# menmitsu/opticalFlowClustering

Measured on AMD Instinct MI355X. Metric: Mpixels/s dense flow+kmeans @1080p, higher is better.
Workload: dtype f32 storage, f64 accumulation; 1 GPU; BASELINE.json configs[2]: 300-frame 1080p synthetic clip, Farneback flow (0.5,3,15,3,5,1.2,0) + Lloyd k=5 over (u,v), frames sharded over 1 GPU(s); width=1920, height=1080, frames=300, pairs=299, k=5, lloyd_iters=11, flow_batch_pairs=64

## Files before the change

include/ofc.h:

```cpp
#ifndef OFC_H
#define OFC_H
#include <stddef.h>
#include <stdint.h>

#ifdef __cplusplus
extern "C" {
#endif

#define OFC_VERSION 100

enum {
    OFC_OK = 0,
    OFC_EINVAL = -1,
    OFC_ENODEV = -2,
    OFC_EHIP = -3,
    OFC_ENOMEM = -4,
    OFC_ENOTREADY = -5,
    OFC_EUNSUPPORTED = -6,
    OFC_ECOMM = -7
};

enum { OFC_U8 = 0, OFC_F32 = 1, OFC_F64 = 2 };

int ofc_version(void);
const char *ofc_last_error(void);
int ofc_device_count(int *n);

int ofc_malloc(int device, size_t bytes, void **dptr);
int ofc_free(int device, void *dptr);
int ofc_memcpy_h2d(int device, void *dst_dev, const void *src_host, size_t bytes);
int ofc_memcpy_d2h(int device, void *dst_host, const void *src_dev, size_t bytes);
int ofc_memset(int device, void *dst_dev, int value, size_t bytes);
int ofc_device_sync(int device);

typedef struct ofc_fb_params {
    double pyr_scale;
    int levels;
    int winsize;
    int iterations;
    int poly_n;
    double poly_sigma;
    int flags;
} ofc_fb_params;
#define OFC_WINSIZE_MAX 255

void ofc_fb_default_params(ofc_fb_params *p);

typedef struct ofc_flow ofc_flow_t;

int ofc_flow_create(int device, int W, int H, const ofc_fb_params *p, int max_batch,
                    ofc_flow_t **out);
void ofc_flow_destroy(ofc_flow_t *f);

int ofc_flow_calc(ofc_flow_t *f, const uint8_t *prev_gray, const uint8_t *next_gray,
                  float *flow_out);

int ofc_flow_calc_frames_dev(ofc_flow_t *f, const uint8_t *frames_dev, int n_frames,
                             float *flow_dev);
int ofc_flow_calc_frames_dev_stats(ofc_flow_t *f, const uint8_t *frames_dev, int n_frames,
                                   float *flow_dev, double *uv_sum_dev);
int ofc_flow_sync(ofc_flow_t *f);

int ofc_flow_push_gray(ofc_flow_t *f, const uint8_t *gray, float *flow_out);

int ofc_flow_push_bgr(ofc_flow_t *f, const uint8_t *bgr, uint8_t *vis_out, float *mean_mag,
                      float *flow_out);
int ofc_flow_last_vis_dev(ofc_flow_t *f, const uint8_t **vis_dev);

int ofc_level_image(int device, const uint8_t *gray, int W, int H, const ofc_fb_params *p, int k,
                    float *out, int *w_out, int *h_out);
int ofc_polyexp(int device, const float *img, int W, int H, int n, double sigma, float *R5);
int ofc_polyexp_u8(int device, const uint8_t *gray, int W, int H, int n, double sigma, float *R5);
int ofc_update_matrices(int device, const float *R0, const float *R1, const float *flow, int W,
                        int H, float *M);
int ofc_box_solve(int device, const float *M, int W, int H, int winsize, float *flow);
int ofc_flow_resize(int device, const float *flow, int sw, int sh, int dw, int dh, float mul,
                    float *out);

int ofc_flow_iterate(int device, const float *R0, const float *R1, const float *flow_in, int W, int H,
                     int winsize, int iters, int mode, int rows_per_block, float *flow_out);
int ofc_flow_launch_geometry(int W, int H, int n_pairs, int winsize, int out[3]);
int ofc_bench_flow_iters(int device, int W, int H, int n_pairs, int reps, int mode, float *ms);

int ofc_bench_polyexp(int device, int W, int H, int n_images, int iters, int rows_per_block,
                      float *ms_per_launch);

int ofc_bgr2gray(int device, const uint8_t *bgr, int W, int H, uint8_t *gray);
int ofc_flow_to_bgr(int device, const float *flow, int W, int H, uint8_t *bgr, float *mean_mag);
int ofc_flow_to_bgr_dev(int device, const float *flow_dev, int W, int H, int n_frames,
                        uint8_t *bgr_dev, float *mean_mag_dev);
int ofc_bgr2hsv(int device, const uint8_t *bgr, int64_t npix, uint8_t *hsv);
int ofc_preprocess_rgba(int device, const uint8_t *img3, int64_t npix, int thresh, uint8_t *rgba);
int ofc_grid_cell_means(int device, const uint8_t *bgr, int W, int H, int rows, int cols,
                        uint8_t *mean_bgr, uint8_t *hsv);

int ofc_kmeans_fit(int device, const void *X, int dtype, int64_t N, int d, int k,
                   const double *init, int max_iter, double tol_rel, double *centers,
                   int32_t *labels, double *inertia, int *n_iter);
int ofc_kmeans_predict(int device, const void *X, int dtype, int64_t N, int d, int k,
                       const double *centers, int32_t *labels);
int ofc_kmeans_fit_dev(int device, const void *X_dev, int dtype, int64_t N, int d, int k,
                       const double *init, int max_iter, double tol_rel, double *centers,
                       uint8_t *labels_dev, double *inertia, int *n_iter);
int ofc_kmeans_fit_dev_stats(int device, const void *X_dev, int dtype, int64_t N, int d, int k,
                             const double *init, int max_iter, double tol_rel, const double *colsum,
                             double *centers, uint8_t *labels_dev, double *inertia, int *n_iter);
int ofc_kmeans_fit_dev_field(int device, const void *X_dev, int dtype, int64_t N, int d, int k,
                             const double *init, int max_iter, double tol_rel, const double *colsum,
                             double *centers, uint8_t *labels_dev, double *inertia, int *n_iter,
                             int W, int H, int64_t n_fields);
int64_t ofc_lloyd_field_origin(int64_t tile, int quad, int W);
int ofc_lloyd_field_origins(int64_t tile0, int64_t n_tiles, int W, int64_t *out);
void ofc_lloyd_field_shape(int *tile_w, int *tile_h, int *group_w, int *group_h);
int ofc_lloyd_prune_stats(int device, double *out6);
int ofc_bench_lloyd_sweep(int device, const float *X_dev, int64_t N, int k, const double *centers, const double *mean,
                          int what, int iters, float *ms_per_launch);
int ofc_lloyd_colstats_dev(int device, const void *X_dev, int dtype, int64_t N, int d, const double *mean,
                           int pass, double *out);
int ofc_lloyd_step_dev(int device, const void *X_dev, int dtype, int64_t N, int d, int k, const double *mean,
                       const double *centers_c, uint8_t *labels_dev, int accumulate, double *record);
int ofc_lloyd_inertia_dev(int device, const void *X_dev, int dtype, int64_t N, int d, int k, const double *mean,
                          const double *centers_c, const uint8_t *labels_dev, double *inertia);
int ofc_lloyd_farthest_dev(int device, const void *X_dev, int dtype, int64_t N, int d, int k, const double *mean,
                           const double *centers_c, const uint8_t *labels_dev, const int64_t *excl, int n_excl,
                           double *dist2, int64_t *index, double *x_c, int *label);

int ofc_kmeans_fit_w(int device, const void *X, int dtype, const void *w, int w_dtype, int64_t N, int d, int k,
                     const double *init, int max_iter, double tol_rel, double *centers, int32_t *labels,
                     double *inertia, int *n_iter);
int ofc_kmeans_fit_dev_w(int device, const void *X_dev, int dtype, const void *w_dev, int w_dtype, int64_t N, int d,
                         int k, const double *init, int max_iter, double tol_rel, const double *colsum,
                         double *centers, uint8_t *labels_dev, double *inertia, int *n_iter);
int ofc_kmeans_score(int device, const void *X, int dtype, const void *w, int w_dtype, int64_t N, int d, int k,
                     const double *centers, double *inertia);
int ofc_lloyd_step_dev_w(int device, const void *X_dev, int dtype, const void *w_dev, int w_dtype, int64_t N, int d,
                         int k, const double *mean, const double *centers_c, uint8_t *labels_dev, double *record);
int ofc_lloyd_inertia_dev_w(int device, const void *X_dev, int dtype, const void *w_dev, int w_dtype, int64_t N, int d,
                            int k, const double *mean, const double *centers_c, const uint8_t *labels_dev,
                            double *inertia);
int ofc_lloyd_farthest_dev_w(int device, const void *X_dev, int dtype, const void *w_dev, int w_dtype, int64_t N, int d,
                             int k, const double *mean, const double *centers_c, const uint8_t *labels_dev,
                             const int64_t *excl, int n_excl, double *dist2, int64_t *index, double *x_c, int *label,
                             double *weight);
int ofc_flow_weights_dev(int device, const float *flow_dev, int64_t n, int kind, float thr, float *w_dev);
// ... 173 lines not shown
```

opticalflowclustering_amd/_lib.py:

```python
import ctypes as C
import os

import numpy as np

_HERE = os.path.dirname(os.path.abspath(__file__))
LIB_PATH = os.path.join(_HERE, "libofc.so")

OFC_OK, OFC_EINVAL, OFC_ENODEV, OFC_EHIP, OFC_ENOMEM, OFC_ENOTREADY, OFC_EUNSUPPORTED, OFC_ECOMM = \
    0, -1, -2, -3, -4, -5, -6, -7
U8, F32, F64 = 0, 1, 2
UNIQUE_ID_BYTES = 128
KPP_CHUNK = 1024
UV_HIST_SHARE = 2048
UV_HIST_MAX_GRID = 2048
BLOB_TILE_W, BLOB_TILE_H, BLOB_FIELDS = 64, 16, 12
BLOB_LINK_FIELDS, BLOB_NO_MOVE = 3, -0x7fff8000
CONSIST_OK, CONSIST_MISMATCH, CONSIST_LEAVES, CONSIST_INVALID, CONSIST_STATES = 0, 1, 2, 3, 4
CONSIST_SHARE, CONSIST_MAX_DIM = 2048, 16384
CONSIST_ALPHA_MAX, CONSIST_BETA_MAX = 65536, 1 << 62
PHOTO_SHARE, PHOTO_TAU_MAX, PHOTO_KAPPA_MAX, PHOTO_NSTAT = 2048, 65280, 1024, 5
REPAIR_ROUNDS_MAX, REPAIR_NCOUNT, REPAIR_UNFILLED = 254, 3, 255


class OfcError(RuntimeError):
    def __init__(self, code, msg):
        super().__init__(f"libofc error {code}: {msg}")
        self.code = code


class FbParams(C.Structure):
    _fields_ = [("pyr_scale", C.c_double), ("levels", C.c_int), ("winsize", C.c_int),
                ("iterations", C.c_int), ("poly_n", C.c_int), ("poly_sigma", C.c_double),
                ("flags", C.c_int)]

    def __init__(self, pyr_scale=0.5, levels=3, winsize=15, iterations=3, poly_n=5, poly_sigma=1.2,
                 flags=0):
        super().__init__(pyr_scale, levels, winsize, iterations, poly_n, poly_sigma, flags)


_lib = None

_vp, _i, _i64, _f, _d, _sz = C.c_void_p, C.c_int, C.c_int64, C.c_float, C.c_double, C.c_size_t
_ip = C.POINTER(C.c_int)
_PROTOS = {
    "ofc_version": ([], _i),
    "ofc_last_error": ([], C.c_char_p),
    "ofc_device_count": ([_ip], _i),
    "ofc_malloc": ([_i, _sz, C.POINTER(_vp)], _i),
    "ofc_free": ([_i, _vp], _i),
    "ofc_memcpy_h2d": ([_i, _vp, _vp, _sz], _i),
    "ofc_memcpy_d2h": ([_i, _vp, _vp, _sz], _i),
    "ofc_memset": ([_i, _vp, _i, _sz], _i),
    "ofc_device_sync": ([_i], _i),
    "ofc_fb_default_params": ([C.POINTER(FbParams)], None),
    "ofc_flow_create": ([_i, _i, _i, C.POINTER(FbParams), _i, C.POINTER(_vp)], _i),
    "ofc_flow_destroy": ([_vp], None),
    "ofc_flow_calc": ([_vp, _vp, _vp, _vp], _i),
    "ofc_flow_calc_frames_dev": ([_vp, _vp, _i, _vp], _i),
    "ofc_flow_calc_frames_dev_stats": ([_vp, _vp, _i, _vp, _vp], _i),
    "ofc_flow_sync": ([_vp], _i),
    "ofc_flow_push_gray": ([_vp, _vp, _vp], _i),
    "ofc_flow_push_bgr": ([_vp, _vp, _vp, C.POINTER(_f), _vp], _i),
    "ofc_flow_last_vis_dev": ([_vp, C.POINTER(_vp)], _i),
    "ofc_level_image": ([_i, _vp, _i, _i, C.POINTER(FbParams), _i, _vp, _ip, _ip], _i),
    "ofc_polyexp": ([_i, _vp, _i, _i, _i, _d, _vp], _i),
    "ofc_polyexp_u8": ([_i, _vp, _i, _i, _i, _d, _vp], _i),
    "ofc_update_matrices": ([_i, _vp, _vp, _vp, _i, _i, _vp], _i),
    "ofc_box_solve": ([_i, _vp, _i, _i, _i, _vp], _i),
    "ofc_flow_resize": ([_i, _vp, _i, _i, _i, _i, _f, _vp], _i),
    "ofc_flow_iterate": ([_i, _vp, _vp, _vp, _i, _i, _i, _i, _i, _i, _vp], _i),
    "ofc_flow_launch_geometry": ([_i, _i, _i, _i, _ip], _i),
    "ofc_bench_flow_iters": ([_i, _i, _i, _i, _i, _i, C.POINTER(_f)], _i),
    "ofc_bench_polyexp": ([_i, _i, _i, _i, _i, _i, C.POINTER(_f)], _i),
    "ofc_bgr2gray": ([_i, _vp, _i, _i, _vp], _i),
    "ofc_flow_to_bgr": ([_i, _vp, _i, _i, _vp, C.POINTER(_f)], _i),
    "ofc_flow_to_bgr_dev": ([_i, _vp, _i, _i, _i, _vp, _vp], _i),
    "ofc_bgr2hsv": ([_i, _vp, _i64, _vp], _i),
    "ofc_preprocess_rgba": ([_i, _vp, _i64, _i, _vp], _i),
    "ofc_grid_cell_means": ([_i, _vp, _i, _i, _i, _i, _vp, _vp], _i),
    "ofc_kmeans_fit": ([_i, _vp, _i, _i64, _i, _i, _vp, _i, _d, _vp, _vp, C.POINTER(_d), _ip], _i),
    "ofc_kmeans_predict": ([_i, _vp, _i, _i64, _i, _i, _vp, _vp], _i),
    "ofc_kmeans_fit_dev": ([_i, _vp, _i, _i64, _i, _i, _vp, _i, _d, _vp, _vp, C.POINTER(_d), _ip], _i),
    "ofc_kmeans_fit_dev_stats": ([_i, _vp, _i, _i64, _i, _i, _vp, _i, _d, _vp, _vp, _vp, C.POINTER(_d), _ip], _i),
    "ofc_kmeans_fit_dev_field": ([_i, _vp, _i, _i64, _i, _i, _vp, _i, _d, _vp, _vp, _vp, C.POINTER(_d), _ip, _i, _i, _i64], _i),
    "ofc_lloyd_field_origin": ([_i64, _i, _i], _i64),
    "ofc_lloyd_field_origins": ([_i64, _i64, _i, _vp], _i),
    "ofc_lloyd_field_shape": ([_ip, _ip, _ip, _ip], None),
    "ofc_lloyd_prune_stats": ([_i, _vp], _i),
    "ofc_bench_lloyd_sweep": ([_i, _vp, _i64, _i, _vp, _vp, _i, _i, C.POINTER(_f)], _i),
    "ofc_lloyd_colstats_dev": ([_i, _vp, _i, _i64, _i, _vp, _i, _vp], _i),
    "ofc_lloyd_step_dev": ([_i, _vp, _i, _i64, _i, _i, _vp, _vp, _vp, _i, _vp], _i),
    "ofc_lloyd_inertia_dev": ([_i, _vp, _i, _i64, _i, _i, _vp, _vp, _vp, C.POINTER(_d)], _i),
    "ofc_lloyd_farthest_dev": ([_i, _vp, _i, _i64, _i, _i, _vp, _vp, _vp, _vp, _i, C.POINTER(_d), C.POINTER(_i64), _vp, _ip], _i),
    "ofc_kmeans_fit_w": ([_i, _vp, _i, _vp, _i, _i64, _i, _i, _vp, _i, _d, _vp, _vp, C.POINTER(_d), _ip], _i),
    "ofc_kmeans_fit_dev_w": ([_i, _vp, _i, _vp, _i, _i64, _i, _i, _vp, _i, _d, _vp, _vp, _vp, C.POINTER(_d), _ip], _i),
    "ofc_kmeans_score": ([_i, _vp, _i, _vp, _i, _i64, _i, _i, _vp, C.POINTER(_d)], _i),
    "ofc_lloyd_step_dev_w": ([_i, _vp, _i, _vp, _i, _i64, _i, _i, _vp, _vp, _vp, _vp], _i),
    "ofc_lloyd_inertia_dev_w": ([_i, _vp, _i, _vp, _i, _i64, _i, _i, _vp, _vp, _vp, C.POINTER(_d)], _i),
    "ofc_lloyd_farthest_dev_w": ([_i, _vp, _i, _vp, _i, _i64, _i, _i, _vp, _vp, _vp, _vp, _i, C.POINTER(_d), C.POINTER(_i64), _vp, _ip,
                                  C.POINTER(_d)], _i),
    "ofc_flow_weights_dev": ([_i, _vp, _i64, _i, _f, _vp], _i),
    "ofc_bench_lloyd_sweep_w": ([_i, _vp, _vp, _i, _i64, _i, _vp, _vp, _i, C.POINTER(_f)], _i),
    "ofc_kpp_candidates": ([_i, _vp, _i, _i64, _i, _vp, _vp, _i, _vp, _vp, _vp], _i),
    "ofc_kpp_seed_dev": ([_i, _vp, _i, _i64, _i, _i, _vp, _i64, _vp, _i, _vp, _vp], _i),
    "ofc_kpp_sample_dev": ([_i, _vp, _i64, _vp, _i, _vp], _i),
    "ofc_kpp_seed_dev_w": ([_i, _vp, _i, _vp, _i, _i64, _i, _i, _vp, _d, _vp, _i, _vp, _vp], _i),
    "ofc_kpp_sample_dev_w": ([_i, _vp, _i, _vp, _i64, _vp, _i, _i, _vp, _vp], _i),
    "ofc_kmeans_fit_batched": ([_i, _vp, _vp, _i, _i, _i, _vp, _i, _d, _vp, _vp, _vp, _vp], _i),
    "ofc_grid_kmeans": ([_i, _vp, _i, _i, _i, _i, _i, _vp, _i, _d, _i, _vp, _vp], _i),
    "ofc_grid_kmeans_dev": ([_i, _vp, _i, _i, _i, _i, _i, _i, _vp, _i, _d, _i, _vp, _vp], _i),
    "ofc_dist_unique_id": ([_vp], _i),
    "ofc_dist_init": ([_i, _i, _i, _vp], _i),
    "ofc_dist_allreduce_f64": ([_i, _vp, _i], _i),
    "ofc_dist_init_host": ([_i, _i, _i, _vp, _vp], _i),
    "ofc_dist_loopback": ([_i], _i),
    "ofc_dist_finalize": ([], _i),
    "ofc_stream_create": ([_i, _i, _i, C.POINTER(FbParams), _i, _i, _i, C.POINTER(_vp)], _i),
    "ofc_stream_push_gray": ([_vp, _vp, _ip], _i),
    "ofc_stream_finish": ([_vp, _vp, _i, _ip], _i),
    "ofc_stream_set_model": ([_vp, _i, _vp, _vp, _i], _i),
    "ofc_stream_finish_clusters": ([_vp, _vp, _vp, _vp, _i, _ip], _i),
    "ofc_stream_set_histogram": ([_vp, _i, _f], _i),
    "ofc_stream_read_histogram": ([_vp, _vp, _i], _i),
    "ofc_stream_destroy": ([_vp], None),
    "ofc_grid_cell_mean_flow": ([_i, _vp, _i, _i, _i, _i, _vp], _i),
    "ofc_grid_label_counts_dev": ([_i, _vp, _vp, _i, _i, _i, _i, _i, _i, _vp, _vp], _i),
    "ofc_grid_assign_counts_dev": ([_i, _vp, _i, _i, _i, _i, _i, _i, _vp, _vp, _vp, _vp], _i),
    "ofc_uv_hist_accum_dev": ([_i, _vp, _i64, _i, _f, _vp], _i),
    "ofc_uv_hist": ([_i, _vp, _i64, _i, _f, _vp], _i),
    "ofc_bench_uv_hist": ([_i, _vp, _i64, _i, _f, _i, C.POINTER(_f)], _i),
    "ofc_motion_check": ([_i, _i, _i], _i),
    "ofc_motion_launch_geometry": ([_i, _i, _i, _ip], _i),
    "ofc_motion_solve": ([_vp, _i, _vp, _ip], _i),
    "ofc_motion_moments_dev": ([_i, _vp, _i, _i, _i, _vp, _vp, _vp], _i),
    "ofc_motion_fit_dev": ([_i, _vp, _i, _i, _i, _i, _vp, _i, _vp, _vp, _vp, _vp], _i),
    "ofc_motion_subtract_dev": ([_i, _vp, _i, _i, _i, _vp, _vp], _i),
    "ofc_motion_fit": ([_i, _vp, _i, _i, _i, _i, _vp, _i, _vp, _vp, _vp, _vp], _i),
    "ofc_motion_compensate": ([_i, _vp, _i, _i, _i, _i, _vp, _i, _vp, _vp, _vp, _vp, _vp], _i),
    "ofc_stream_set_camera": ([_vp, _i, _vp, _i], _i),
    "ofc_stream_read_camera": ([_vp, _vp, _vp, _i], _i),
    "ofc_bench_motion": ([_i, _vp, _i, _i, _i, _i, _i, C.POINTER(_f)], _i),
    "ofc_blob_check": ([_i, _i, _i, _i, _i, _i], _i),
    "ofc_blob_keys_dev": ([_i, _vp, _i, _i, _i, _i, _f, _i, _vp, _vp, C.c_uint32, _i, _vp], _i),
# ... 108 lines not shown
```

opticalflowclustering_amd/csrc/ofc_api.cpp:

```cpp
#include "color_common.h"
#include "lloyd_common.h"

#include <cfloat>
#include <algorithm>
#include <cmath>
#include <cstdlib>
#include <memory>

namespace ofc {

static thread_local std::string g_err;

void set_error(const char *fmt, ...)
{
    char buf[1024];
    va_list ap;
    va_start(ap, fmt);
    vsnprintf(buf, sizeof(buf), fmt, ap);
    va_end(ap);
    g_err = buf;
}

int ensure_device(int device)
{
// ... 109 lines not shown
        set_error("winsize %d unsupported (odd 5..%d)", p.winsize, OFC_WINSIZE_MAX);
        return OFC_EUNSUPPORTED;
    }
    return polyexp_n_check(p.poly_n);
}

}

using namespace ofc;

extern "C" {

int ofc_version(void) { return OFC_VERSION; }
const char *ofc_last_error(void) { return g_err.c_str(); }

int ofc_device_count(int *n)
{
    OFC_REQUIRE(n, "null pointer");
    int c = 0;
    hipError_t e = hipGetDeviceCount(&c);
    *n = (e == hipSuccess) ? c : 0;
    return OFC_OK;
}

int ofc_malloc(int device, size_t bytes, void **dptr)
{
    OFC_REQUIRE(dptr, "null pointer");
    OFC_TRY(ensure_device(device));
    OFC_HIP(hipMalloc(dptr, bytes));
    return OFC_OK;
}

int ofc_free(int device, void *dptr)
{
    OFC_TRY(ensure_device(device));
    OFC_HIP(hipFree(dptr));
    return OFC_OK;
}

int ofc_memcpy_h2d(int device, void *dst, const void *src, size_t bytes)
{
    OFC_TRY(ensure_device(device));
    OFC_HIP(hipMemcpy(dst, src, bytes, hipMemcpyHostToDevice));
    return OFC_OK;
}

int ofc_memcpy_d2h(int device, void *dst, const void *src, size_t bytes)
{
    OFC_TRY(ensure_device(device));
    OFC_HIP(hipMemcpy(dst, src, bytes, hipMemcpyDeviceToHost));
    return OFC_OK;
}

int ofc_memset(int device, void *dst, int value, size_t bytes)
{
    OFC_TRY(ensure_device(device));
    OFC_HIP(hipMemset(dst, value, bytes));
    return OFC_OK;
}

int ofc_device_sync(int device)
{
    OFC_TRY(ensure_device(device));
    OFC_HIP(hipDeviceSynchronize());
    return OFC_OK;
}

void ofc_fb_default_params(ofc_fb_params *p)
{
    if (!p) return;
    p->pyr_scale = 0.5; p->levels = 3; p->winsize = 15; p->iterations = 3;
    p->poly_n = 5; p->poly_sigma = 1.2; p->flags = 0;
}

}

struct ofc_flow {
    int device = 0, W = 0, H = 0, max_batch = 0, levels = 0;
    ofc_fb_params prm{};
    PolyConsts pc{};
    std::vector<LevelGeom> geom;
    hipStream_t stream = nullptr;
    DevBuf I, R, M, flowA, flowB, flowC;
    bool fused = true;
    bool fuse_level0 = true;
    bool fuse2 = false;
    int fuse2_min_w = 0;
    bool w3 = false;
    int w3_min_w = 0;
    DevBuf frames2, flow1;
    DevBuf prev_gray;
    bool have_prev = false;
    DevBuf bgr_in, vis, vis_partial, vis_stats, mean_mag;
    bool have_vis = false;
    DevBuf uv_scratch;
    struct Captured {
        const uint8_t *frames = nullptr;
        int n_frames = 0;
        float *flow = nullptr;
        double *uv_sum = nullptr;
        int hits = 0;
        hipGraph_t graph = nullptr;
        hipGraphExec_t exec = nullptr;
    };
    std::vector<Captured> graphs;
    bool use_graph = false;
};

namespace ofc {

static int flow_run(ofc_flow *f, const uint8_t *frames_dev, int n_frames, float *flow_dev, double *uv_sum_dev = nullptr)
{
    const int npair = n_frames - 1;
    const int W = f->W, H = f->H;
    hipStream_t s = f->stream;
    float *I = f->I.as<float>(), *R = f->R.as<float>();
    const int iters = f->prm.iterations;
    float *prevFlow = nullptr;
    int pw = 0, ph = 0;
    for (int k = f->levels; k >= 0; k--) {
        const LevelGeom &g = f->geom[k];
        const size_t P = (size_t)g.w * g.h;
        float *dst = (k == 0) ? flow_dev : (((f->levels - k) & 1) ? f->flowB.as<float>() : f->flowA.as<float>());
        float *tmp = f->flowC.as<float>();
        if (k == 0 && f->fuse_level0 && polyexp_u8_ok(W, H, g)) {
            OFC_TRY(launch_polyexp_u8(frames_dev, R, n_frames, W, H, f->pc, s));
        } else {
            OFC_TRY(launch_level_image(frames_dev, I, n_frames, W, H, g, s));
            OFC_TRY(launch_polyexp(I, R, n_frames, g.w, g.h, f->pc, 0, s));
        }
        const size_t strideR = 5 * P;
        const float mul = (float)(1. / f->prm.pyr_scale);
        if (f->fused) {
            const bool two = f->fuse2 && f->prm.winsize == 15 && g.w >= f->fuse2_min_w;
            int plan[64], L = 0;
            for (int i = 0; i < iters;) {
                const int n = (two && i > 0 && iters - i >= 2) ? 2 : 1;
                plan[L++] = n;
                i += n;
            }
            const float *cur = nullptr;
            for (int l = 0; l < L; l++) {
                float *nxt = ((L - 1 - l) & 1) ? tmp : dst;
                if (l == 0 && prevFlow) {
                    OFC_TRY(launch_flow_iter(R, strideR, nullptr, nxt, npair, g.w, g.h, f->prm.winsize, s, prevFlow, pw, ph, mul));
                } else {
                    if (l == 0) {
                        float *z = (nxt == dst) ? tmp : dst;
                        OFC_HIP(hipMemsetAsync(z, 0, sizeof(float) * 2 * P * npair, s));
                        cur = z;
                    }
                    if (uv_sum_dev && k == 0 && l == L - 1 && plan[l] == 1 && f->prm.winsize == 15 && !(f->w3 && g.w >= f->w3_min_w)) {
                        const size_t need = (size_t)flow_iter_max_grid(g.w, g.h, npair, f->prm.winsize) * 2;
                        if (f->uv_scratch.bytes < need * sizeof(double)) OFC_TRY(f->uv_scratch.alloc(need * sizeof(double)));
                        OFC_TRY(launch_flow_iter(R, strideR, cur, nxt, npair, g.w, g.h, f->prm.winsize, s, nullptr, 0, 0, 1.f,
                                                 uv_sum_dev, f->uv_scratch.as<double>(), f->uv_scratch.bytes / sizeof(double)));
                        uv_sum_dev = nullptr;
                    } else
                    if (plan[l] == 2) OFC_TRY(launch_flow_iter2(R, strideR, cur, nxt, npair, g.w, g.h, f->prm.winsize, s));
                    else if (f->w3 && f->prm.winsize == 15 && g.w >= f->w3_min_w)
                        OFC_TRY(launch_flow_iter_w3(R, strideR, cur, nxt, npair, g.w, g.h, f->prm.winsize, s));
                    else OFC_TRY(launch_flow_iter(R, strideR, cur, nxt, npair, g.w, g.h, f->prm.winsize, s));
                }
                cur = nxt;
            }
        } else {
            float *cur = dst;
            if (!prevFlow) {
                OFC_HIP(hipMemsetAsync(cur, 0, sizeof(float) * 2 * P * npair, s));
            } else {
                OFC_TRY(launch_flow_resize(prevFlow, cur, npair, pw, ph, g.w, g.h, mul, s));
            }
            float *M = f->M.as<float>();
            OFC_TRY(launch_update_matrices(R, R + strideR, strideR, cur, M, npair, g.w, g.h, s));
            for (int i = 0; i < iters; i++) {
                OFC_TRY(launch_box_solve(M, cur, npair, g.w, g.h, f->prm.winsize, 0, s));
                if (i < iters - 1)
                    OFC_TRY(launch_update_matrices(R, R + strideR, strideR, cur, M, npair, g.w, g.h, s));
            }
        }
        prevFlow = dst;
        pw = g.w; ph = g.h;
    }
    if (uv_sum_dev) {
        const int64_t N = (int64_t)npair * W * H;
        const int max_blocks = 1024;
        const int nblocks = (int)std::max<int64_t>(1, std::min<int64_t>(cdiv64(N / 4, 256), max_blocks));
        if (f->uv_scratch.bytes < sizeof(double) * 2 * max_blocks) OFC_TRY(f->uv_scratch.alloc(sizeof(double) * 2 * max_blocks));
        OFC_TRY(launch_lloyd_colstats(flow_dev, OFC_F32, N, 2, nullptr, 0, f->uv_scratch.as<double>(), nblocks, s));
        OFC_TRY(launch_reduce_records(f->uv_scratch.as<double>(), nblocks, 2, uv_sum_dev, s));
    }
    return OFC_OK;
}

static int flow_run_cached(ofc_flow *f, const uint8_t *frames_dev, int n_frames, float *flow_dev, double *uv_sum_dev)
{
    if (!f->use_graph) return flow_run(f, frames_dev, n_frames, flow_dev, uv_sum_dev);
    ofc_flow::Captured *c = nullptr;
    for (auto &g : f->graphs)
        if (g.frames == frames_dev && g.n_frames == n_frames && g.flow == flow_dev && g.uv_sum == uv_sum_dev) { c = &g; break; }
    if (!c) {
        if (f->graphs.size() >= 64) {
            for (auto &g : f->graphs) {
                if (g.exec) (void)hipGraphExecDestroy(g.exec);
                if (g.graph) (void)hipGraphDestroy(g.graph);
            }
            f->graphs.clear();
        }
        f->graphs.emplace_back();
        c = &f->graphs.back();
        c->frames = frames_dev; c->n_frames = n_frames; c->flow = flow_dev; c->uv_sum = uv_sum_dev;
    }
    c->hits++;
    if (c->exec) {
        OFC_HIP(hipGraphLaunch(c->exec, f->stream));
        return OFC_OK;
    }
    if (c->hits < 2) return flow_run(f, frames_dev, n_frames, flow_dev, uv_sum_dev);
    OFC_HIP(hipStreamBeginCapture(f->stream, hipStreamCaptureModeThreadLocal));
    const int rc = flow_run(f, frames_dev, n_frames, flow_dev, uv_sum_dev);
    hipGraph_t g = nullptr;
    const hipError_t e = hipStreamEndCapture(f->stream, &g);
    if (rc != OFC_OK || e != hipSuccess || !g) {
        if (g) (void)hipGraphDestroy(g);
        f->use_graph = false;
        (void)hipGetLastError();
        return flow_run(f, frames_dev, n_frames, flow_dev, uv_sum_dev);
    }
    hipGraphExec_t ex = nullptr;
    if (hipGraphInstantiate(&ex, g, nullptr, nullptr, 0) != hipSuccess || !ex) {
        (void)hipGraphDestroy(g);
        f->use_graph = false;
        (void)hipGetLastError();
        return flow_run(f, frames_dev, n_frames, flow_dev, uv_sum_dev);
    }
    c->graph = g;
    c->exec = ex;
    OFC_HIP(hipGraphLaunch(c->exec, f->stream));
    return OFC_OK;
}

}

extern "C" {

int ofc_flow_create(int device, int W, int H, const ofc_fb_params *p, int max_batch, ofc_flow_t **out)
{
    OFC_REQUIRE(out, "null out pointer");
    *out = nullptr;
    ofc_fb_params prm;
    if (p) prm = *p; else ofc_fb_default_params(&prm);
    OFC_TRY(check_params(prm, W, H));
    OFC_REQUIRE(max_batch >= 1 && max_batch <= 4096, "max_batch out of range");
    OFC_REQUIRE((prm.winsize & 1) && prm.winsize >= 5, "winsize must be odd and >= 5");
    std::unique_ptr<ofc_flow> f(new ofc_flow);
    f->device = device; f->W = W; f->H = H; f->max_batch = max_batch; f->prm = prm;
    f->levels = pyramid_levels(W, H, prm);
    for (int k = 0; k <= f->levels; k++) f->geom.push_back(level_geometry(W, H, prm, k));
    {
        const char *e = getenv("OFC_FLOW_STAGED");
        f->fused = prm.winsize <= 15 && !(e && e[0] == '1');
        f->fuse_level0 = !(e && e[0] == '1');
        const char *e3 = getenv("OFC_FLOW_W3");
        if (e3 && e3[0]) {
            const int v = atoi(e3);
            f->w3 = v != 0;
            f->w3_min_w = v > 1 ? v : 0;
        }
        const char *eg = getenv("OFC_FLOW_GRAPH");
        f->use_graph = eg && eg[0] == '1';
        const char *e2 = getenv("OFC_FLOW_FUSE2");
        if (e2 && e2[0]) {
            const int v = atoi(e2);
            f->fuse2 = v != 0;
            if (v > 1) f->fuse2_min_w = v;
        }
    }
    OFC_TRY(flow_levels_check(W, H, prm, f->geom.data(), f->levels, f->fused, f->fuse_level0));
    OFC_TRY(ensure_device(device));
    polyexp_setup(prm.poly_n, prm.poly_sigma, f->pc);
    OFC_HIP(hipStreamCreateWithFlags(&f->stream, hipStreamNonBlocking));
    const size_t P0 = (size_t)W * H, nb = (size_t)max_batch;
    OFC_TRY(f->I.alloc(sizeof(float) * P0 * (nb + 1)));
    OFC_TRY(f->R.alloc(sizeof(float) * 5 * P0 * (nb + 1)));
    if (f->fused) {
        OFC_TRY(f->flowC.alloc(sizeof(float) * 2 * P0 * nb));
    } else {
        OFC_TRY(f->M.alloc(sizeof(float) * 5 * P0 * nb));
    }
    const size_t P1 = f->levels >= 1 ? (size_t)f->geom[1].w * f->geom[1].h : 1;
    OFC_TRY(f->flowA.alloc(sizeof(float) * 2 * P1 * nb));
    OFC_TRY(f->flowB.alloc(sizeof(float) * 2 * P1 * nb));
    OFC_TRY(f->frames2.alloc(2 * P0));
    OFC_TRY(f->flow1.alloc(sizeof(float) * 2 * P0));
    OFC_TRY(f->prev_gray.alloc(P0));
    *out = f.release();
    return OFC_OK;
}

void ofc_flow_destroy(ofc_flow_t *f)
{
    if (!f) return;
    (void)hipSetDevice(f->device);
    if (f->stream) {
        (void)hipStreamSynchronize(f->stream);
        (void)hipStreamDestroy(f->stream);
    }
    for (auto &g : f->graphs) {
        if (g.exec) (void)hipGraphExecDestroy(g.exec);
        if (g.graph) (void)hipGraphDestroy(g.graph);
    }
    delete f;
}

int ofc_flow_calc_frames_dev(ofc_flow_t *f, const uint8_t *frames_dev, int n_frames, float *flow_dev)
{
    OFC_REQUIRE(f && frames_dev && flow_dev, "null pointer");
    OFC_REQUIRE(n_frames >= 2 && n_frames - 1 <= f->max_batch, "n_frames-1 = %d pairs not in [1, max_batch=%d]",
                n_frames - 1, f->max_batch);
    OFC_TRY(ensure_device(f->device));
    return flow_run_cached(f, frames_dev, n_frames, flow_dev, nullptr);
}

int ofc_flow_calc_frames_dev_stats(ofc_flow_t *f, const uint8_t *frames_dev, int n_frames, float *flow_dev, double *uv_sum_dev)
{
    OFC_REQUIRE(f && frames_dev && flow_dev && uv_sum_dev, "null pointer");
    OFC_REQUIRE(n_frames >= 2 && n_frames - 1 <= f->max_batch, "n_frames-1 = %d pairs not in [1, max_batch=%d]",
                n_frames - 1, f->max_batch);
    OFC_TRY(ensure_device(f->device));
    return flow_run_cached(f, frames_dev, n_frames, flow_dev, uv_sum_dev);
}

hipStream_t ofc_flow_stream_internal(ofc_flow_t *f) { return f->stream; }

int ofc_flow_sync(ofc_flow_t *f)
{
    OFC_REQUIRE(f, "null pointer");
    OFC_TRY(ensure_device(f->device));
    OFC_HIP(hipStreamSynchronize(f->stream));
    return OFC_OK;
}

int ofc_flow_calc(ofc_flow_t *f, const uint8_t *prev_gray, const uint8_t *next_gray, float *flow_out)
{
    OFC_REQUIRE(f && prev_gray && next_gray && flow_out, "null pointer");
    OFC_TRY(ensure_device(f->device));
    const size_t P0 = (size_t)f->W * f->H;
    uint8_t *fr = f->frames2.as<uint8_t>();
    OFC_HIP(hipMemcpyAsync(fr, prev_gray, P0, hipMemcpyHostToDevice, f->stream));
    OFC_HIP(hipMemcpyAsync(fr + P0, next_gray, P0, hipMemcpyHostToDevice, f->stream));
    OFC_TRY(flow_run(f, fr, 2, f->flow1.as<float>()));
    OFC_HIP(hipMemcpyAsync(flow_out, f->flow1.p, sizeof(float) * 2 * P0, hipMemcpyDeviceToHost, f->stream));
    OFC_HIP(hipStreamSynchronize(f->stream));
    return OFC_OK;
}

int ofc_flow_push_gray(ofc_flow_t *f, const uint8_t *gray, float *flow_out)
{
    OFC_REQUIRE(f && gray, "null pointer");
    OFC_TRY(ensure_device(f->device));
    const size_t P0 = (size_t)f->W * f->H;
    uint8_t *fr = f->frames2.as<uint8_t>();
    if (!f->have_prev) {
        OFC_HIP(hipMemcpyAsync(f->prev_gray.p, gray, P0, hipMemcpyHostToDevice, f->stream));
        OFC_HIP(hipStreamSynchronize(f->stream));
        f->have_prev = true;
        set_error("first frame pushed: no pair yet");
        return OFC_ENOTREADY;
    }
    OFC_REQUIRE(flow_out, "null flow_out");
    OFC_HIP(hipMemcpyAsync(fr, f->prev_gray.p, P0, hipMemcpyDeviceToDevice, f->stream));
    OFC_HIP(hipMemcpyAsync(fr + P0, gray, P0, hipMemcpyHostToDevice, f->stream));
    OFC_HIP(hipMemcpyAsync(f->prev_gray.p, fr + P0, P0, hipMemcpyDeviceToDevice, f->stream));
    OFC_TRY(flow_run(f, fr, 2, f->flow1.as<float>()));
    OFC_HIP(hipMemcpyAsync(flow_out, f->flow1.p, sizeof(float) * 2 * P0, hipMemcpyDeviceToHost, f->stream));
    OFC_HIP(hipStreamSynchronize(f->stream));
    return OFC_OK;
}

int ofc_flow_push_bgr(ofc_flow_t *f, const uint8_t *bgr, uint8_t *vis_out, float *mean_mag, float *flow_out)
{
    OFC_REQUIRE(f && bgr, "null pointer");
    OFC_TRY(ensure_device(f->device));
    const size_t P0 = (size_t)f->W * f->H;
    hipStream_t s = f->stream;
    if (!f->bgr_in.p) {
        OFC_TRY(f->bgr_in.alloc(P0 * 3 + 16));
        OFC_TRY(f->vis.alloc(P0 * 3 + 16));
        OFC_TRY(f->vis_partial.alloc(sizeof(double) * 3 * VIS_BLOCKS));
        OFC_TRY(f->vis_stats.alloc(sizeof(VisFrameStats)));
        OFC_TRY(f->mean_mag.alloc(sizeof(float)));
    }
    uint8_t *fr = f->frames2.as<uint8_t>();
    OFC_HIP(hipMemcpyAsync(f->bgr_in.p, bgr, P0 * 3, hipMemcpyHostToDevice, s));
    if (!f->have_prev) {
        OFC_TRY(launch_bgr2gray(f->bgr_in.as<uint8_t>(), f->prev_gray.as<uint8_t>(), (int64_t)P0, s));
        OFC_HIP(hipStreamSynchronize(s));
        f->have_prev = true;
        set_error("first frame pushed: no pair yet");
        return OFC_ENOTREADY;
    }
    OFC_HIP(hipMemcpyAsync(fr, f->prev_gray.p, P0, hipMemcpyDeviceToDevice, s));
    OFC_TRY(launch_bgr2gray(f->bgr_in.as<uint8_t>(), fr + P0, (int64_t)P0, s));
    OFC_HIP(hipMemcpyAsync(f->prev_gray.p, fr + P0, P0, hipMemcpyDeviceToDevice, s));
    OFC_TRY(flow_run(f, fr, 2, f->flow1.as<float>()));
    OFC_TRY(launch_flow_to_bgr(f->flow1.as<float>(), f->W, f->H, 1, f->vis.as<uint8_t>(), f->mean_mag.as<float>(),
                               f->vis_partial.as<double>(), f->vis_stats.as<VisFrameStats>(), s));
    if (vis_out) OFC_HIP(hipMemcpyAsync(vis_out, f->vis.p, P0 * 3, hipMemcpyDeviceToHost, s));
    if (mean_mag) OFC_HIP(hipMemcpyAsync(mean_mag, f->mean_mag.p, sizeof(float), hipMemcpyDeviceToHost, s));
    if (flow_out) OFC_HIP(hipMemcpyAsync(flow_out, f->flow1.p, sizeof(float) * 2 * P0, hipMemcpyDeviceToHost, s));
    OFC_HIP(hipStreamSynchronize(s));
    f->have_vis = true;
    return OFC_OK;
}

int ofc_flow_last_vis_dev(ofc_flow_t *f, const uint8_t **vis_dev)
{
    OFC_REQUIRE(f && vis_dev, "null pointer");
    OFC_REQUIRE(f->have_vis, "no visualisation yet: no ofc_flow_push_bgr has returned OFC_OK");
    *vis_dev = f->vis.as<uint8_t>();
    return OFC_OK;
}
// ... 275 lines not shown
```

opticalflowclustering_amd/flow.py:

```python
import ctypes as C
import threading
from collections import OrderedDict

import numpy as np

from . import _lib
from ._lib import FbParams, check, load, ptr


class FlowEngine:

    def __init__(self, W, H, params=None, max_batch=1, device=0):
        self.W, self.H, self.device, self.max_batch = int(W), int(H), device, int(max_batch)
        self.params = params or FbParams()
        h = C.c_void_p()
        check(load().ofc_flow_create(device, self.W, self.H, C.byref(self.params), self.max_batch, C.byref(h)))
        self._h = h

    def calc(self, prev_gray, next_gray, out=None):
        prev_gray = np.ascontiguousarray(prev_gray, np.uint8)
        next_gray = np.ascontiguousarray(next_gray, np.uint8)
        if prev_gray.shape != (self.H, self.W) or next_gray.shape != (self.H, self.W):
            raise ValueError(f"expected two {self.H}x{self.W} uint8 images")
        if out is None:
            out = np.empty((self.H, self.W, 2), np.float32)
        elif not _is_flow_buffer(out, self.H, self.W):
            raise ValueError(f"out must be a writeable C-contiguous {self.H}x{self.W}x2 float32 array")
        check(load().ofc_flow_calc(self._h, ptr(prev_gray), ptr(next_gray), ptr(out)))
        return out

    def push(self, gray):
        gray = np.ascontiguousarray(gray, np.uint8)
        if gray.shape != (self.H, self.W):
            raise ValueError(f"expected a {self.H}x{self.W} uint8 image")
        flow = np.empty((self.H, self.W, 2), np.float32)
        rc = load().ofc_flow_push_gray(self._h, ptr(gray), ptr(flow))
        if rc == _lib.OFC_ENOTREADY:
            return None
        check(rc)
        return flow

    def calc_frames_dev(self, frames_ptr, n_frames, flow_ptr, sync=True, uv_sum_ptr=None):
        if uv_sum_ptr:
            check(load().ofc_flow_calc_frames_dev_stats(self._h, C.c_void_p(frames_ptr), n_frames, C.c_void_p(flow_ptr),
                                                        C.c_void_p(uv_sum_ptr)))
        else:
            check(load().ofc_flow_calc_frames_dev(self._h, C.c_void_p(frames_ptr), n_frames, C.c_void_p(flow_ptr)))
        if sync:
            self.sync()

    def sync(self):
        check(load().ofc_flow_sync(self._h))

    def close(self):
        if getattr(self, "_h", None):
            load().ofc_flow_destroy(self._h)
            self._h = None

    def __del__(self):
        try:
            self.close()
        except Exception:
            pass


def _is_flow_buffer(a, H, W):
    return (isinstance(a, np.ndarray) and a.dtype == np.float32 and a.shape == (H, W, 2)
            and a.flags.c_contiguous and a.flags.writeable)


OPTFLOW_USE_INITIAL_FLOW = 4
OPTFLOW_FARNEBACK_GAUSSIAN = 256

_FB_CACHE_MAX = 4
_fb_engines = OrderedDict()
_fb_lock = threading.Lock()


def _gray_arg(a, name):
    if not isinstance(a, np.ndarray) or a.dtype != np.uint8 or a.ndim != 2:
        raise ValueError(f"{name} must be a 2-D uint8 array (one grey frame)")
    return np.ascontiguousarray(a)


def calcOpticalFlowFarneback(prev, next, flow, pyr_scale, levels, winsize, iterations, poly_n, poly_sigma, flags,
                             device=0):
    prev = _gray_arg(prev, "prev")
    next = _gray_arg(next, "next")
    if prev.shape != next.shape:
        raise ValueError(f"prev {prev.shape} and next {next.shape} differ in shape")
    H, W = prev.shape
    out = flow if _is_flow_buffer(flow, H, W) else np.empty((H, W, 2), np.float32)
    key = (int(device), W, H, float(pyr_scale), int(levels), int(winsize), int(iterations), int(poly_n),
           float(poly_sigma), int(flags))
    with _fb_lock:
        eng = _fb_engines.get(key)
        if eng is None:
            eng = FlowEngine(W, H, FbParams(*key[3:]), max_batch=1, device=key[0])
            _fb_engines[key] = eng
            while len(_fb_engines) > _FB_CACHE_MAX:
                _fb_engines.popitem(last=False)[1].close()
        else:
            _fb_engines.move_to_end(key)
        eng.calc(prev, next, out)
    return out


def clear_farneback_cache():
    with _fb_lock:
        while _fb_engines:
            _fb_engines.popitem()[1].close()
```

Before: 18570 Mpixels/s.

## Overlap coarse pyramid level image and polyexp on a side stream

Gives each pyramid level its own I/R buffers so the level-image and polynomial-expansion work for coarse levels runs on a second stream while the main stream does level-0 polyexp and the coarse-to-fine flow iterations. Events make each level's solve wait for its front end. The aim is to hide front-end latency and fill idle CUs during small coarse-level kernels. The cost is extra memory, bounded by a 1.5x cap, plus event overhead, and the path is turned off when graphs are in use.

```diff
diff --git a/include/ofc.h b/include/ofc.h
--- a/include/ofc.h
+++ b/include/ofc.h
@@ -60,6 +60,7 @@
 int ofc_flow_calc_frames_dev_stats(ofc_flow_t *f, const uint8_t *frames_dev, int n_frames,
                                    float *flow_dev, double *uv_sum_dev);
 int ofc_flow_sync(ofc_flow_t *f);
+int ofc_flow_front_overlap(const ofc_flow_t *f, int *on);
 
 int ofc_flow_push_gray(ofc_flow_t *f, const uint8_t *gray, float *flow_out);
 
diff --git a/opticalflowclustering_amd/_lib.py b/opticalflowclustering_amd/_lib.py
--- a/opticalflowclustering_amd/_lib.py
+++ b/opticalflowclustering_amd/_lib.py
@@ -59,6 +59,7 @@
     "ofc_flow_calc_frames_dev": ([_vp, _vp, _i, _vp], _i),
     "ofc_flow_calc_frames_dev_stats": ([_vp, _vp, _i, _vp, _vp], _i),
     "ofc_flow_sync": ([_vp], _i),
+    "ofc_flow_front_overlap": ([_vp, _ip], _i),
     "ofc_flow_push_gray": ([_vp, _vp, _vp], _i),
     "ofc_flow_push_bgr": ([_vp, _vp, _vp, C.POINTER(_f), _vp], _i),
     "ofc_flow_last_vis_dev": ([_vp, C.POINTER(_vp)], _i),
diff --git a/opticalflowclustering_amd/csrc/ofc_api.cpp b/opticalflowclustering_amd/csrc/ofc_api.cpp
--- a/opticalflowclustering_amd/csrc/ofc_api.cpp
+++ b/opticalflowclustering_amd/csrc/ofc_api.cpp
@@ -215,6 +215,11 @@
     std::vector<LevelGeom> geom;
     hipStream_t stream = nullptr;
     DevBuf I, R, M, flowA, flowB, flowC;
+    bool front_overlap = false;
+    hipStream_t side = nullptr;
+    hipEvent_t fork = nullptr;
+    std::vector<hipEvent_t> ready;
+    std::vector<size_t> offI, offR;
     bool fused = true;
     bool fuse_level0 = true;
     bool fuse2 = false;
@@ -247,20 +252,35 @@
     const int npair = n_frames - 1;
     const int W = f->W, H = f->H;
     hipStream_t s = f->stream;
-    float *I = f->I.as<float>(), *R = f->R.as<float>();
     const int iters = f->prm.iterations;
     float *prevFlow = nullptr;
     int pw = 0, ph = 0;
+    auto front_end = [&](int k, hipStream_t st) -> int {
+        float *I = f->I.as<float>() + f->offI[k], *R = f->R.as<float>() + f->offR[k];
+        const LevelGeom &g = f->geom[k];
+        if (k == 0 && f->fuse_level0 && polyexp_u8_ok(W, H, g)) return launch_polyexp_u8(frames_dev, R, n_frames, W, H, f->pc, st);
+        OFC_TRY(launch_level_image(frames_dev, I, n_frames, W, H, g, st));
+        return launch_polyexp(I, R, n_frames, g.w, g.h, f->pc, 0, st);
+    };
+    if (f->front_overlap) {
+        OFC_HIP(hipEventRecord(f->fork, s));
+        OFC_HIP(hipStreamWaitEvent(f->side, f->fork, 0));
+        for (int k = f->levels; k >= 1; k--) {
+            OFC_TRY(front_end(k, f->side));
+            OFC_HIP(hipEventRecord(f->ready[k], f->side));
+        }
+        OFC_TRY(front_end(0, s));
+    }
     for (int k = f->levels; k >= 0; k--) {
         const LevelGeom &g = f->geom[k];
         const size_t P = (size_t)g.w * g.h;
         float *dst = (k == 0) ? flow_dev : (((f->levels - k) & 1) ? f->flowB.as<float>() : f->flowA.as<float>());
         float *tmp = f->flowC.as<float>();
-        if (k == 0 && f->fuse_level0 && polyexp_u8_ok(W, H, g)) {
-            OFC_TRY(launch_polyexp_u8(frames_dev, R, n_frames, W, H, f->pc, s));
-        } else {
-            OFC_TRY(launch_level_image(frames_dev, I, n_frames, W, H, g, s));
-            OFC_TRY(launch_polyexp(I, R, n_frames, g.w, g.h, f->pc, 0, s));
+        const float *R = f->R.as<float>() + f->offR[k];
+        if (!f->front_overlap) {
+            OFC_TRY(front_end(k, s));
+        } else if (k >= 1) {
+            OFC_HIP(hipStreamWaitEvent(s, f->ready[k], 0));
         }
         const size_t strideR = 5 * P;
         const float mul = (float)(1. / f->prm.pyr_scale);
@@ -386,7 +406,7 @@
     OFC_TRY(check_params(prm, W, H));
     OFC_REQUIRE(max_batch >= 1 && max_batch <= 4096, "max_batch out of range");
     OFC_REQUIRE((prm.winsize & 1) && prm.winsize >= 5, "winsize must be odd and >= 5");
-    std::unique_ptr<ofc_flow> f(new ofc_flow);
+    std::unique_ptr<ofc_flow, void (*)(ofc_flow_t *)> f(new ofc_flow, ofc_flow_destroy);
     f->device = device; f->W = W; f->H = H; f->max_batch = max_batch; f->prm = prm;
     f->levels = pyramid_levels(W, H, prm);
     for (int k = 0; k <= f->levels; k++) f->geom.push_back(level_geometry(W, H, prm, k));
@@ -414,8 +434,35 @@
     polyexp_setup(prm.poly_n, prm.poly_sigma, f->pc);
     OFC_HIP(hipStreamCreateWithFlags(&f->stream, hipStreamNonBlocking));
     const size_t P0 = (size_t)W * H, nb = (size_t)max_batch;
-    OFC_TRY(f->I.alloc(sizeof(float) * P0 * (nb + 1)));
-    OFC_TRY(f->R.alloc(sizeof(float) * 5 * P0 * (nb + 1)));
+    size_t nI = P0 * (nb + 1), nR = 5 * P0 * (nb + 1);
+    f->offI.assign(f->levels + 1, 0);
+    f->offR.assign(f->levels + 1, 0);
+    {
+        const bool u8_level0 = f->fuse_level0 && polyexp_u8_ok(W, H, f->geom[0]);
+        std::vector<size_t> oI(f->levels + 1, 0), oR(f->levels + 1, 0);
+        size_t sI = 0, sR = 0;
+        for (int k = 0; k <= f->levels; k++) {
+            const size_t Pk = (size_t)f->geom[k].w * f->geom[k].h;
+            oR[k] = sR;
+            sR += (5 * Pk * (nb + 1) + 63) & ~(size_t)63;
+            oI[k] = sI;
+            if (k > 0 || !u8_level0) sI += (Pk * (nb + 1) + 63) & ~(size_t)63;
+        }
+        const char *eo = getenv("OFC_FLOW_FRONT_OVERLAP");
+        f->front_overlap = !(eo && eo[0] == '0') && f->levels >= 1 && !f->use_graph && 2 * (sI + sR) <= 3 * (nI + nR);
+        if (f->front_overlap) {
+            f->offI = oI; f->offR = oR;
+            nI = sI; nR = sR;
+        }
+    }
+    if (f->front_overlap) {
+        OFC_HIP(hipStreamCreateWithFlags(&f->side, hipStreamNonBlocking));
+        OFC_HIP(hipEventCreateWithFlags(&f->fork, hipEventDisableTiming));
+        f->ready.assign(f->levels + 1, nullptr);
+        for (int k = 1; k <= f->levels; k++) OFC_HIP(hipEventCreateWithFlags(&f->ready[k], hipEventDisableTiming));
+    }
+    OFC_TRY(f->I.alloc(sizeof(float) * nI));
+    OFC_TRY(f->R.alloc(sizeof(float) * nR));
     if (f->fused) {
         OFC_TRY(f->flowC.alloc(sizeof(float) * 2 * P0 * nb));
     } else {
@@ -434,11 +481,14 @@
 void ofc_flow_destroy(ofc_flow_t *f)
 {
     if (!f) return;
-    (void)hipSetDevice(f->device);
-    if (f->stream) {
-        (void)hipStreamSynchronize(f->stream);
-        (void)hipStreamDestroy(f->stream);
-    }
+    if (f->stream) (void)hipSetDevice(f->device);
+    for (hipStream_t s : {f->stream, f->side})
+        if (s) (void)hipStreamSynchronize(s);
+    for (hipStream_t s : {f->stream, f->side})
+        if (s) (void)hipStreamDestroy(s);
+    if (f->fork) (void)hipEventDestroy(f->fork);
+    for (hipEvent_t e : f->ready)
+        if (e) (void)hipEventDestroy(e);
     for (auto &g : f->graphs) {
         if (g.exec) (void)hipGraphExecDestroy(g.exec);
         if (g.graph) (void)hipGraphDestroy(g.graph);
@@ -471,6 +521,13 @@
     OFC_REQUIRE(f, "null pointer");
     OFC_TRY(ensure_device(f->device));
     OFC_HIP(hipStreamSynchronize(f->stream));
+    return OFC_OK;
+}
+
+int ofc_flow_front_overlap(const ofc_flow_t *f, int *on)
+{
+    OFC_REQUIRE(f && on, "null pointer");
+    *on = f->front_overlap ? 1 : 0;
     return OFC_OK;
 }
 
diff --git a/opticalflowclustering_amd/flow.py b/opticalflowclustering_amd/flow.py
--- a/opticalflowclustering_amd/flow.py
+++ b/opticalflowclustering_amd/flow.py
@@ -51,6 +51,11 @@
 
     def sync(self):
         check(load().ofc_flow_sync(self._h))
+
+    def front_overlap(self):
+        on = C.c_int(-1)
+        check(load().ofc_flow_front_overlap(self._h, C.byref(on)))
+        return bool(on.value)
 
     def close(self):
         if getattr(self, "_h", None):
```

Measured after the change: 19050 Mpixels/s, median of 6. 2.6% higher.
